# ZeningLin/ViBERTgrid-PyTorch

Measured on AMD Instinct MI355X. Metric: training docs/sec, 512x512 img + seq_len 512, bert-base+resnet34; 1/2/4/8 GPU, higher is better.
Workload: dtype f32

## Files before the change

vibertgrid-pytorch_amd/csrc/gemm_planes.hip:

```cpp
#include "vbg_common.h"
#include <type_traits>
#include <cstdlib>
#include <hip/hip_ext.h>
#include "../../include/vbg.h"

namespace vbg {

typedef unsigned pg_u32x4 __attribute__((ext_vector_type(4)));
typedef __bf16 pg_bf16x8 __attribute__((ext_vector_type(8)));
constexpr unsigned PG_INVALID = 0x80000000u;

__device__ __forceinline__ __amdgpu_buffer_rsrc_t pg_rsrc(const void* base) {
    return __builtin_amdgcn_make_buffer_rsrc(const_cast<void*>(base), 0, (int)0x80000000u, 0x00020000);
}

typedef _Float16 pg_f16x8 __attribute__((ext_vector_type(8)));
__device__ __forceinline__ void pg_split2(float a, float b, unsigned& hi, unsigned& lo) {
    typedef float f32x2_t __attribute__((ext_vector_type(2)));
    typedef _Float16 f16x2_t __attribute__((ext_vector_type(2)));
    const f32x2_t v = {a, b};
    const f16x2_t h = __builtin_convertvector(v, f16x2_t);
    const f16x2_t l = __builtin_convertvector((v - __builtin_convertvector(h, f32x2_t)) * 2048.f, f16x2_t);
    hi = __builtin_bit_cast(unsigned, h);
    lo = __builtin_bit_cast(unsigned, l);
// ... 336 lines not shown
            mma(fa1, fb1);
            __builtin_amdgcn_sched_barrier(0);
            asm volatile("s_waitcnt vmcnt(0) lgkmcnt(0)" ::: "memory");
            __builtin_amdgcn_s_barrier();
            __builtin_amdgcn_sched_barrier(0);
            read_frags(nxt, fo0, fa0, fb0);
        }
        __builtin_amdgcn_sched_barrier(0);
        settle0();
        cur = nxt;
    }
    }
    __syncthreads();

    const float* bias = p.bias;
    const bool add_bias = (bias != nullptr) && (split == 0);
    const int accumulate = p.accumulate, epi = p.epi;
    const bool atomic = accumulate && p.splitk > 1;
    float alpha = p.alpha;
    if constexpr (FORM) { if (a_amax) alpha *= vbg_pow2_scale(vbg_amax_read(a_amax)).y; }
    const long long ldc = ldc_;
    float* const C = pC;
    float* const C2 = p.C2;
    float* const Ct = reinterpret_cast<float*>(smem);
#pragma unroll
    for (int j = 0; j < TN; ++j)
#pragma unroll
        for (int i = 0; i < TM; ++i)
#pragma unroll
            for (int r = 0; r < 16; ++r)
                Ct[(wm * WM + i * 32 + (r & 3) + 8 * (r >> 2) + 4 * lk) * CTS + wn * WN + j * 32 + lr] =
                    (FORM == 1 ? acc[i][j][r] + acx[FORM == 1 ? i : 0][FORM == 1 ? j : 0][r] * (1.f / 2048.f) : acc[i][j][r]) * alpha;
    __syncthreads();
    constexpr int QN = BN / 4;
    unsigned short* const Cp = p.Cp;
    unsigned short* const Cq = p.Cq;
    float vmax = 0.f;
    float qsc = 1.f;
    if (Cq && p.cq_ref_in) {
        const float amx = __uint_as_float(vbg_amax_read(p.cq_ref_in));
        const float l1 = p.cq_l1_in ? __uint_as_float(*p.cq_l1_in) : 1.f;
        const float bound = amx * l1 * p.cq_mul;
        qsc = vbg_pow2_scale(__float_as_uint(bound)).x;
        if (p.cq_ref_out && pid == 0 && tid == 0) p.cq_ref_out[0] = __float_as_uint(bound);
    }
#pragma unroll
    for (int q = 0; q < BM * QN / NT; ++q) {
        const int idx = tid + q * NT;
        const int row = idx / QN, c = (idx % QN) * 4;
        const int gm = m0 + row, gn = n0 + c;
        if (gm >= M || gn >= N) continue;
        float4 v = *reinterpret_cast<const float4*>(&Ct[row * CTS + c]);
        if (add_bias) {
            const float4 b = *reinterpret_cast<const float4*>(bias + gn);
            v.x += b.x; v.y += b.y; v.z += b.z; v.w += b.w;
        }
        float* cp = C + (long long)gm * ldc + gn;
        if (atomic) {
            unsafeAtomicAdd(cp + 0, v.x); unsafeAtomicAdd(cp + 1, v.y); unsafeAtomicAdd(cp + 2, v.z); unsafeAtomicAdd(cp + 3, v.w);
            continue;
        }
        if (accumulate) {
            const float4 o = *reinterpret_cast<const float4*>(cp);
            v.x += o.x; v.y += o.y; v.z += o.z; v.w += o.w;
        }
        if (epi == VBG_EPI_RELU) v = make_float4(fmaxf(v.x, 0.f), fmaxf(v.y, 0.f), fmaxf(v.z, 0.f), fmaxf(v.w, 0.f));
        if (epi == VBG_EPI_MUL_GELU_GRAD) {
            const float4 hv = *reinterpret_cast<const float4*>(C2 + (long long)gm * ldc + gn);
            v.x *= gelu_erf_grad(hv.x); v.y *= gelu_erf_grad(hv.y); v.z *= gelu_erf_grad(hv.z); v.w *= gelu_erf_grad(hv.w);
        }
        if (C) *reinterpret_cast<float4*>(cp) = v;
        vmax = fmaxf(fmaxf(vmax, fmaxf(fabsf(v.x), fabsf(v.y))), fmaxf(fabsf(v.z), fabsf(v.w)));
        if (p.colsum) *reinterpret_cast<float4*>(&Ct[row * CTS + c]) = v;
        if (epi == VBG_EPI_GELU_DUAL) {
            v = make_float4(gelu_erf(v.x), gelu_erf(v.y), gelu_erf(v.z), gelu_erf(v.w));
            if (C2) *reinterpret_cast<float4*>(C2 + (long long)gm * ldc + gn) = v;
        }
        if (Cp) {
            const float e[4] = {v.x, v.y, v.z, v.w};
            unsigned short h[4], m[4], l[4];
#pragma unroll
            for (int t = 0; t < 4; ++t) {
                const unsigned u = __float_as_uint(e[t]);
                const float r1 = e[t] - __uint_as_float(u & 0xffff0000u);
                const unsigned u1 = __float_as_uint(r1);
                const float r2 = r1 - __uint_as_float(u1 & 0xffff0000u);
                h[t] = (unsigned short)(u >> 16); m[t] = (unsigned short)(u1 >> 16); l[t] = (unsigned short)(__float_as_uint(r2) >> 16);
            }
            unsigned short* o = Cp + (long long)gm * p.ldp + gn;
            *reinterpret_cast<uint2*>(o) = make_uint2(h[0] | ((unsigned)h[1] << 16), h[2] | ((unsigned)h[3] << 16));
            *reinterpret_cast<uint2*>(o + p.c_plane) = make_uint2(m[0] | ((unsigned)m[1] << 16), m[2] | ((unsigned)m[3] << 16));
            *reinterpret_cast<uint2*>(o + 2 * p.c_plane) = make_uint2(l[0] | ((unsigned)l[1] << 16), l[2] | ((unsigned)l[3] << 16));
        }
        if (Cq) {
            unsigned short* o = Cq + (long long)gm * p.ldq + gn;
            uint2 h, l;
            pg_split2(v.x * qsc, v.y * qsc, h.x, l.x);
            pg_split2(v.z * qsc, v.w * qsc, h.y, l.y);
            *reinterpret_cast<uint2*>(o) = h;
            *reinterpret_cast<uint2*>(o + p.q_plane) = l;
        }
    }
    if (p.colsum) {
        __syncthreads();
        if (tid < BN && n0 + tid < N) {
            float cs = 0.f;
            const int rows = min(BM, M - m0);
            for (int r = 0; r < rows; ++r) cs += Ct[r * CTS + tid];
            unsafeAtomicAdd(p.colsum + n0 + tid, cs);
        }
    }
    if (p.c_amax) {
        __syncthreads();
        vbg_amax_publish(vmax, p.c_amax, Ct);
    }
}

__device__ __forceinline__ void pg_split3(float x, unsigned short& h, unsigned short& m, unsigned short& l);

__global__ __launch_bounds__(512) void plane_gemm_256_kernel(const vbg_plane_gemm_desc p) {
    constexpr int BM = 256, BN = 256, WGN = 4, NW = 8, NT = 512, NST = 3, BK = 16;
    constexpr int WM = 128, WN = 64, TM = 4, TN = 2;
    constexpr int PA = BM * 32, PB = BN * 32;
    constexpr int STAGE = 3 * (PA + PB);
    constexpr int NIA = 3, NIB = 3;
    constexpr int CTS = BN + 4;
    constexpr int SMEM = NST * STAGE;
    static_assert(64 * CTS * 4 <= SMEM, "epilogue pass fits");
    __shared__ __attribute__((aligned(1024))) unsigned char smem[SMEM];

    const int tid = threadIdx.x, lane = tid & 63, wave = tid >> 6;
    const int M = p.M, N = p.N;
    const long long a_plane = p.a_plane, b_plane = p.b_plane, lda = p.lda, ldb = p.ldb;
    constexpr unsigned XCDS = 8, XCD_GROUP = 8;
    const unsigned gx = gridDim.x, gy = gridDim.y;
    const unsigned lin = blockIdx.x + gridDim.x * blockIdx.y;
    const unsigned total = gx * gy;
    const unsigned xcd = lin % XCDS, local = lin / XCDS;
    const unsigned per_xcd = (total + XCDS - 1) / XCDS, tall = (total % XCDS) ? (total % XCDS) : XCDS;
    const unsigned rem = xcd < tall ? xcd * per_xcd + local : tall * per_xcd + (xcd - tall) * (per_xcd - 1) + local;
    const unsigned band = XCD_GROUP * gy, bid = rem / band, first = bid * XCD_GROUP;
    const unsigned bm = min(gx - first, XCD_GROUP), inb = rem - bid * band;
    const unsigned tile_m = first + inb % bm, tile_n = inb / bm;
    const int m0 = (int)tile_m * BM, n0 = (int)tile_n * BN;
    if (m0 >= M || n0 >= N) return;
    const int ntiles = p.K / BK;

    unsigned avo[NIA], bvo[NIB];
    int alds[NIA], blds[NIB];
    {
        const int lrow = lane >> 1;
#pragma unroll
        for (int i = 0; i < NIA; ++i) {
            const int u = wave + NW * i, q = u / 8, rb = u % 8;
            const int r = rb * 32 + lrow;
            const int half = (lane & 1) ^ ((r >> 3) & 1);
            avo[i] = (m0 + r < M) ? (unsigned)(((long long)q * a_plane + (long long)r * lda) * 2 + half * 16) : PG_INVALID;
            alds[i] = __builtin_amdgcn_readfirstlane(q * PA + rb * 1024);
        }
#pragma unroll
        for (int i = 0; i < NIB; ++i) {
            const int u = wave + NW * i, q = u / 8, rb = u % 8;
            const int r = rb * 32 + lrow;
            const int half = (lane & 1) ^ ((r >> 3) & 1);
            bvo[i] = (n0 + r < N) ? (unsigned)(((long long)q * b_plane + (long long)r * ldb) * 2 + half * 16) : PG_INVALID;
            blds[i] = __builtin_amdgcn_readfirstlane(3 * PA + q * PB + rb * 1024);
        }
    }
    const unsigned short* abase = p.A + (long long)m0 * lda;
    const unsigned short* bbase = p.B + (long long)n0 * ldb;
    typedef __attribute__((address_space(3))) void* lds_ptr;
    auto issue = [&](int stage, unsigned inv) {
        unsigned char* sb = smem + stage * STAGE;
        const __amdgpu_buffer_rsrc_t ra = pg_rsrc(abase), rb = pg_rsrc(bbase);
#pragma unroll
        for (int i = 0; i < NIA; ++i)
            __builtin_amdgcn_raw_ptr_buffer_load_lds(ra, (lds_ptr)(sb + alds[i]), 16, (int)(avo[i] | inv), 0, 0, 0);
#pragma unroll
        for (int i = 0; i < NIB; ++i)
            __builtin_amdgcn_raw_ptr_buffer_load_lds(rb, (lds_ptr)(sb + blds[i]), 16, (int)(bvo[i] | inv), 0, 0, 0);
        abase += BK;
        bbase += BK;
    };

    const int wm = wave / WGN, wn = wave % WGN;
    const int lr = lane & 31, lk = lane >> 5;
    const int fo = lr * 32 + ((lk ^ ((lr >> 3) & 1)) << 4);
    f32x16 acc[TM][TN];
#pragma unroll
    for (int i = 0; i < TM; ++i)
#pragma unroll
        for (int j = 0; j < TN; ++j)
#pragma unroll
            for (int r = 0; r < 16; ++r) acc[i][j][r] = 0.f;
    pg_u32x4 fa[3][TM], fb[3][TN];
    auto read_frags = [&](int stage) {
        const unsigned char* as = smem + stage * STAGE + (wm * WM) * 32 + fo;
        const unsigned char* bs = smem + stage * STAGE + 3 * PA + (wn * WN) * 32 + fo;
        constexpr int order[3] = {2, 0, 1};
#pragma unroll
        for (int o = 0; o < 3; ++o) {
            const int q = order[o];
#pragma unroll
            for (int i = 0; i < TM; ++i) fa[q][i] = *reinterpret_cast<const pg_u32x4*>(as + q * PA + i * 32 * 32);
#pragma unroll
            for (int j = 0; j < TN; ++j) fb[q][j] = *reinterpret_cast<const pg_u32x4*>(bs + q * PB + j * 32 * 32);
        }
    };
    auto mma = [&]() {
        constexpr int qa[6] = {2, 0, 1, 1, 0, 0}, qb[6] = {0, 2, 1, 0, 1, 0};
#pragma unroll
        for (int t = 0; t < 6; ++t)
#pragma unroll
            for (int i = 0; i < TM; ++i)
#pragma unroll
                for (int j = 0; j < TN; ++j)
                    acc[i][j] = __builtin_amdgcn_mfma_f32_32x32x16_bf16(__builtin_bit_cast(pg_bf16x8, fa[qa[t]][i]),
                                                                        __builtin_bit_cast(pg_bf16x8, fb[qb[t]][j]), acc[i][j], 0, 0, 0);
    };
    constexpr int NIW = NIA + NIB;
    issue(0, 0u);
    issue(1, ntiles > 1 ? 0u : PG_INVALID);
    asm volatile("s_waitcnt vmcnt(%0)" ::"n"(NIW) : "memory");
    __builtin_amdgcn_s_barrier();
    int cur = 0;
    for (int t = 0; t < ntiles; ++t) {
        const int nxt = (cur + 1 == NST) ? 0 : cur + 1;
        const int nn = (nxt + 1 == NST) ? 0 : nxt + 1;
        issue(nn, t + 2 < ntiles ? 0u : PG_INVALID);
        read_frags(cur);
        mma();
        asm volatile("s_waitcnt vmcnt(%0) lgkmcnt(0)" ::"n"(NIW) : "memory");
        __builtin_amdgcn_s_barrier();
        cur = nxt;
    }
    __syncthreads();

    const float* bias = p.bias;
    const int epi = p.epi;
    const float alpha = p.alpha;
    const long long ldc = p.ldc;
    float* const C = p.C;
    float* const C2 = p.C2;
    unsigned short* const Cp = p.Cp;
    float* const Ct = reinterpret_cast<float*>(smem);
    constexpr int QN = BN / 4;
#pragma unroll
    for (int ps = 0; ps < 4; ++ps) {
        if (wm == (ps >> 1)) {
#pragma unroll
            for (int ii = 0; ii < 2; ++ii)
#pragma unroll
                for (int j = 0; j < TN; ++j)
#pragma unroll
                    for (int r = 0; r < 16; ++r)
                        Ct[(ii * 32 + (r & 3) + 8 * (r >> 2) + 4 * lk) * CTS + wn * WN + j * 32 + lr] = acc[2 * (ps & 1) + ii][j][r] * alpha;
        }
        __syncthreads();
#pragma unroll
        for (int q = 0; q < 64 * QN / NT; ++q) {
            const int idx = tid + q * NT;
            const int row = idx / QN, c = (idx % QN) * 4;
            const int gm = m0 + ps * 64 + row, gn = n0 + c;
            if (gm >= M || gn >= N) continue;
            float4 v = *reinterpret_cast<const float4*>(&Ct[row * CTS + c]);
            if (bias) {
                const float4 b = *reinterpret_cast<const float4*>(bias + gn);
                v.x += b.x; v.y += b.y; v.z += b.z; v.w += b.w;
            }
            float* cp = C + (long long)gm * ldc + gn;
            if (epi == VBG_EPI_RELU) v = make_float4(fmaxf(v.x, 0.f), fmaxf(v.y, 0.f), fmaxf(v.z, 0.f), fmaxf(v.w, 0.f));
            if (epi == VBG_EPI_MUL_GELU_GRAD) {
                const float4 hv = *reinterpret_cast<const float4*>(C2 + (long long)gm * ldc + gn);
                v.x *= gelu_erf_grad(hv.x); v.y *= gelu_erf_grad(hv.y); v.z *= gelu_erf_grad(hv.z); v.w *= gelu_erf_grad(hv.w);
            }
            if (C) *reinterpret_cast<float4*>(cp) = v;
            if (epi == VBG_EPI_GELU_DUAL) {
                v = make_float4(gelu_erf(v.x), gelu_erf(v.y), gelu_erf(v.z), gelu_erf(v.w));
                if (C2) *reinterpret_cast<float4*>(C2 + (long long)gm * ldc + gn) = v;
            }
            if (Cp) {
                const float e[4] = {v.x, v.y, v.z, v.w};
                unsigned short h[4], m[4], l[4];
#pragma unroll
                for (int t = 0; t < 4; ++t) pg_split3(e[t], h[t], m[t], l[t]);
                unsigned short* o = Cp + (long long)gm * p.ldp + gn;
                *reinterpret_cast<uint2*>(o) = make_uint2(h[0] | ((unsigned)h[1] << 16), h[2] | ((unsigned)h[3] << 16));
                *reinterpret_cast<uint2*>(o + p.c_plane) = make_uint2(m[0] | ((unsigned)m[1] << 16), m[2] | ((unsigned)m[3] << 16));
                *reinterpret_cast<uint2*>(o + 2 * p.c_plane) = make_uint2(l[0] | ((unsigned)l[1] << 16), l[2] | ((unsigned)l[3] << 16));
            }
        }
        __syncthreads();
    }
}

__device__ __forceinline__ void pg_split3(float x, unsigned short& h, unsigned short& m, unsigned short& l) {
    const unsigned u = __float_as_uint(x);
    const float r1 = x - __uint_as_float(u & 0xffff0000u);
    const unsigned u1 = __float_as_uint(r1);
    const float r2 = r1 - __uint_as_float(u1 & 0xffff0000u);
    h = (unsigned short)(u >> 16); m = (unsigned short)(u1 >> 16); l = (unsigned short)(__float_as_uint(r2) >> 16);
}

__global__ __launch_bounds__(256) void split_planes_kernel(const float* __restrict__ x, long long ldx, int rows, int cols,
                                                            unsigned short* __restrict__ out, int ldp, long long plane, int relu,
                                                            float* colsum) {
    extern __shared__ float sh_cols[];
    const int cpr = ldp / 8;
    const long long n = (long long)rows * cpr;
    const long long stride = (long long)gridDim.x * blockDim.x;
    float cs[8] = {0.f, 0.f, 0.f, 0.f, 0.f, 0.f, 0.f, 0.f};
    const long long i0 = (long long)blockIdx.x * blockDim.x + threadIdx.x;
    for (long long i = i0; i < n; i += stride) {
        const int r = (int)(i / cpr), c = (int)(i % cpr) * 8;
        float e[8];
        if (c + 8 <= cols && ((ldx & 3) == 0) && ((((uintptr_t)x) & 15) == 0)) {
            const float4 a = *reinterpret_cast<const float4*>(x + (long long)r * ldx + c);
            const float4 b = *reinterpret_cast<const float4*>(x + (long long)r * ldx + c + 4);
            e[0] = a.x; e[1] = a.y; e[2] = a.z; e[3] = a.w; e[4] = b.x; e[5] = b.y; e[6] = b.z; e[7] = b.w;
        } else {
#pragma unroll
            for (int t = 0; t < 8; ++t) e[t] = (c + t < cols) ? x[(long long)r * ldx + c + t] : 0.f;
        }
        unsigned short h[8], m[8], l[8];
#pragma unroll
        for (int t = 0; t < 8; ++t) {
            cs[t] += e[t];
            pg_split3(relu ? fmaxf(e[t], 0.f) : e[t], h[t], m[t], l[t]);
        }
        unsigned short* o = out + (long long)r * ldp + c;
        auto pack = [](const unsigned short* s) {
            return make_uint4(s[0] | ((unsigned)s[1] << 16), s[2] | ((unsigned)s[3] << 16), s[4] | ((unsigned)s[5] << 16), s[6] | ((unsigned)s[7] << 16));
        };
        *reinterpret_cast<uint4*>(o) = pack(h);
        *reinterpret_cast<uint4*>(o + plane) = pack(m);
        *reinterpret_cast<uint4*>(o + 2 * plane) = pack(l);
    }
    if (colsum) {
        for (int c = threadIdx.x; c < ldp; c += blockDim.x) sh_cols[c] = 0.f;
        __syncthreads();
        if (i0 < n) {
            const int c = (int)(i0 % cpr) * 8;
#pragma unroll
            for (int t = 0; t < 8; ++t) atomicAdd(&sh_cols[c + t], cs[t]);
        }
        __syncthreads();
        for (int c = threadIdx.x; c < cols; c += blockDim.x) {
            const float v = sh_cols[c];
            if (v != 0.f) unsafeAtomicAdd(colsum + c, v);
        }
    }
}

__global__ __launch_bounds__(256) void split_planes_pair_kernel(const float* __restrict__ x, long long ldx, int rows, int cols,
                                                                 unsigned short* __restrict__ out, int ldp, long long plane,
                                                                 const unsigned* amax, float* colsum) {
    extern __shared__ float sh_cols[];
    const float sc = amax ? vbg_pow2_scale(vbg_amax_read(amax)).x : 1.f;
    float cs[8] = {0.f, 0.f, 0.f, 0.f, 0.f, 0.f, 0.f, 0.f};
    const long long i0 = (long long)blockIdx.x * blockDim.x + threadIdx.x;
    const int cpr = ldp / 8;
    const long long n = (long long)rows * cpr;
    const long long stride = (long long)gridDim.x * blockDim.x;
    const bool vec = ((ldx & 3) == 0) && ((((uintptr_t)x) & 15) == 0);
    for (long long i = (long long)blockIdx.x * blockDim.x + threadIdx.x; i < n; i += stride) {
        const int r = (int)(i / cpr), c = (int)(i % cpr) * 8;
        float e[8];
        if (c + 8 <= cols && vec) {
            const float4 a = *reinterpret_cast<const float4*>(x + (long long)r * ldx + c);
            const float4 b = *reinterpret_cast<const float4*>(x + (long long)r * ldx + c + 4);
            e[0] = a.x; e[1] = a.y; e[2] = a.z; e[3] = a.w; e[4] = b.x; e[5] = b.y; e[6] = b.z; e[7] = b.w;
        } else {
#pragma unroll
            for (int t = 0; t < 8; ++t) e[t] = (c + t < cols) ? x[(long long)r * ldx + c + t] : 0.f;
        }
#pragma unroll
        for (int t = 0; t < 8; ++t) { cs[t] += e[t]; e[t] *= sc; }
        uint4 h, l;
        pg_split2(e[0], e[1], h.x, l.x); pg_split2(e[2], e[3], h.y, l.y); pg_split2(e[4], e[5], h.z, l.z); pg_split2(e[6], e[7], h.w, l.w);
        unsigned short* o = out + (long long)r * ldp + c;
        *reinterpret_cast<uint4*>(o) = h;
        *reinterpret_cast<uint4*>(o + plane) = l;
    }
    if (colsum) {
        for (int c = threadIdx.x; c < ldp; c += blockDim.x) sh_cols[c] = 0.f;
        __syncthreads();
        if (i0 < n) {
            const int c = (int)(i0 % cpr) * 8;
#pragma unroll
            for (int t = 0; t < 8; ++t) atomicAdd(&sh_cols[c + t], cs[t]);
        }
        __syncthreads();
        for (int c = threadIdx.x; c < cols; c += blockDim.x) {
            const float v = sh_cols[c];
            if (v != 0.f) unsafeAtomicAdd(colsum + c, v);
        }
    }
}

__global__ __launch_bounds__(256) void col_l1_max_kernel(const vbg_l1_entry* __restrict__ tab, unsigned* __restrict__ out) {
    const vbg_l1_entry e = tab[blockIdx.y];
    const int c0 = blockIdx.x * 64;
    if (c0 >= e.cols) return;
    const int tx = threadIdx.x & 15, ty = threadIdx.x >> 4;
    const int c = c0 + tx * 4;
    const bool vec = (e.ld & 3) == 0 && ((((uintptr_t)e.w) & 15) == 0) && c + 4 <= e.cols;
    float4 s = make_float4(0.f, 0.f, 0.f, 0.f);
#pragma unroll 4
    for (int r = ty; r < e.rows; r += 16) {
        const float* p = e.w + (long long)r * e.ld + c;
        if (vec) {
            const float4 v = *reinterpret_cast<const float4*>(p);
            s.x += fabsf(v.x); s.y += fabsf(v.y); s.z += fabsf(v.z); s.w += fabsf(v.w);
        } else {
            if (c < e.cols) s.x += fabsf(p[0]);
            if (c + 1 < e.cols) s.y += fabsf(p[1]);
            if (c + 2 < e.cols) s.z += fabsf(p[2]);
            if (c + 3 < e.cols) s.w += fabsf(p[3]);
        }
    }
    __shared__ float4 red[16][16];
    red[ty][tx] = s;
    __syncthreads();
    if (ty == 0) {
        float4 t = red[0][tx];
#pragma unroll
        for (int g = 1; g < 16; ++g) { const float4 v = red[g][tx]; t.x += v.x; t.y += v.y; t.z += v.z; t.w += v.w; }
        float m = fmaxf(fmaxf(t.x, t.y), fmaxf(t.z, t.w));
#pragma unroll
        for (int o = 8; o > 0; o >>= 1) m = fmaxf(m, __shfl_xor(m, o, 64));
        if (tx == 0) atomicMax(out + blockIdx.y, __float_as_uint(m));
    }
}

__global__ __launch_bounds__(256) void split_planes_t_kernel(const float* __restrict__ x, long long ldx, int rows, int cols,
                                                              unsigned short* __restrict__ out, int ldp, long long plane) {
    __shared__ float t[64][65];
    const int r0 = blockIdx.x * 64, c0 = blockIdx.y * 64;
    const int tid = threadIdx.x;
    const bool vec = ((ldx & 3) == 0) && ((((uintptr_t)x) & 15) == 0);
#pragma unroll
    for (int i = 0; i < 4; ++i) {
        const int f = tid + i * 256, r = f / 16, c = (f % 16) * 4;
        float4 v = make_float4(0.f, 0.f, 0.f, 0.f);
        if (r0 + r < rows) {
            const float* src = x + (long long)(r0 + r) * ldx + c0 + c;
            if (vec && c0 + c + 4 <= cols) v = *reinterpret_cast<const float4*>(src);
            else {
                if (c0 + c + 0 < cols) v.x = src[0];
                if (c0 + c + 1 < cols) v.y = src[1];
                if (c0 + c + 2 < cols) v.z = src[2];
                if (c0 + c + 3 < cols) v.w = src[3];
            }
        }
        t[r][c] = v.x; t[r][c + 1] = v.y; t[r][c + 2] = v.z; t[r][c + 3] = v.w;
    }
    __syncthreads();
#pragma unroll
    for (int i = 0; i < 2; ++i) {
        const int f = tid + i * 256, c = f / 8, rg = (f % 8) * 8;
        if (c0 + c >= cols || r0 + rg >= ldp) continue;
        unsigned short h[8], m[8], l[8];
#pragma unroll
        for (int e = 0; e < 8; ++e) pg_split3(t[rg + e][c], h[e], m[e], l[e]);
        unsigned short* o = out + (long long)(c0 + c) * ldp + r0 + rg;
        auto pack = [](const unsigned short* s) {
            return make_uint4(s[0] | ((unsigned)s[1] << 16), s[2] | ((unsigned)s[3] << 16), s[4] | ((unsigned)s[5] << 16), s[6] | ((unsigned)s[7] << 16));
        };
        *reinterpret_cast<uint4*>(o) = pack(h);
        *reinterpret_cast<uint4*>(o + plane) = pack(m);
        *reinterpret_cast<uint4*>(o + 2 * plane) = pack(l);
    }
}

template <bool PAIR>
__global__ __launch_bounds__(256) void split_planes_t_batched_kernel(const float* __restrict__ src, unsigned short* __restrict__ dst,
                                                                      const long long* __restrict__ tbl, int njobs, long long plane) {
    __shared__ float t[64][65];
    int j = 0;
    while (j + 1 < njobs && (long long)blockIdx.x >= tbl[(j + 1) * 6 + 5]) ++j;
    const long long* e = tbl + j * 6;
    const float* x = src + e[0];
    const int rows = (int)e[1], cols = (int)e[2], ldp = (int)e[4];
    unsigned short* out = dst + e[3];
    const int local = (int)(blockIdx.x - e[5]);
    const int tr = (ldp + 63) / 64;
    const int r0 = (local % tr) * 64, c0 = (local / tr) * 64;
    const int tid = threadIdx.x;
    const long long ldx = cols;
#pragma unroll
    for (int i = 0; i < 4; ++i) {
        const int f = tid + i * 256, r = f / 16, c = (f % 16) * 4;
        float v[4] = {0.f, 0.f, 0.f, 0.f};
        if (r0 + r < rows) {
#pragma unroll
            for (int q = 0; q < 4; ++q)
                if (c0 + c + q < cols) v[q] = x[(long long)(r0 + r) * ldx + c0 + c + q];
        }
        t[r][c] = v[0]; t[r][c + 1] = v[1]; t[r][c + 2] = v[2]; t[r][c + 3] = v[3];
    }
    __syncthreads();
#pragma unroll
    for (int i = 0; i < 2; ++i) {
        const int f = tid + i * 256, c = f / 8, rg = (f % 8) * 8;
        if (c0 + c >= cols || r0 + rg >= ldp) continue;
        unsigned short* o = out + (long long)(c0 + c) * ldp + r0 + rg;
        if constexpr (PAIR) {
            uint4 h, l;
            pg_split2(t[rg + 0][c], t[rg + 1][c], h.x, l.x); pg_split2(t[rg + 2][c], t[rg + 3][c], h.y, l.y);
            pg_split2(t[rg + 4][c], t[rg + 5][c], h.z, l.z); pg_split2(t[rg + 6][c], t[rg + 7][c], h.w, l.w);
            *reinterpret_cast<uint4*>(o) = h;
            *reinterpret_cast<uint4*>(o + plane) = l;
            continue;
        }
        unsigned short h[8], m[8], l[8];
#pragma unroll
        for (int q = 0; q < 8; ++q) pg_split3(t[rg + q][c], h[q], m[q], l[q]);
        auto pack = [](const unsigned short* s) {
            return make_uint4(s[0] | ((unsigned)s[1] << 16), s[2] | ((unsigned)s[3] << 16), s[4] | ((unsigned)s[5] << 16), s[6] | ((unsigned)s[7] << 16));
        };
        *reinterpret_cast<uint4*>(o) = pack(h);
        *reinterpret_cast<uint4*>(o + plane) = pack(m);
        *reinterpret_cast<uint4*>(o + 2 * plane) = pack(l);
    }
}

template <int BM, int BN, int WGM, int WGN, int NST, bool TRANS = false, int FORM = 1>
static void pg_launch_pair(const vbg_plane_gemm_desc& d, hipStream_t s, hipEvent_t e0, hipEvent_t e1) {
    dim3 g(cdiv(d.M, BM), cdiv(d.N, BN), 1);
    if (d.ngroups > 0) {
        int total = 0;
        for (int i = 0; i < d.ngroups; ++i) total += d.grp[i].tiles_m * d.grp[i].tiles_n;
        g = dim3(total, 1, 1);
    }
    (void)hipGetLastError();
    if (e0 && e1) hipExtLaunchKernelGGL((plane_gemm_kernel<BM, BN, WGM, WGN, NST, TRANS, FORM>), g, dim3(WGM * WGN * 64), 0, s, e0, e1, 0, d);
    else hipLaunchKernelGGL((plane_gemm_kernel<BM, BN, WGM, WGN, NST, TRANS, FORM>), g, dim3(WGM * WGN * 64), 0, s, d);
}

template <int BM, int BN, int WGM, int WGN, int NST, bool TRANS = false>
static void pg_launch(const vbg_plane_gemm_desc& d, hipStream_t s, hipEvent_t e0, hipEvent_t e1) {
    dim3 g(cdiv(d.M, BM), cdiv(d.N, BN), d.splitk);
    if (d.ngroups > 0) {
        int total = 0;
        for (int i = 0; i < d.ngroups; ++i) total += d.grp[i].tiles_m * d.grp[i].tiles_n;
        g = dim3(total, 1, d.splitk);
    }
    (void)hipGetLastError();
    if (e0 && e1) hipExtLaunchKernelGGL((plane_gemm_kernel<BM, BN, WGM, WGN, NST, TRANS>), g, dim3(WGM * WGN * 64), 0, s, e0, e1, 0, d);
    else hipLaunchKernelGGL((plane_gemm_kernel<BM, BN, WGM, WGN, NST, TRANS>), g, dim3(WGM * WGN * 64), 0, s, d);
}

}

using namespace vbg;

static int plane_gemm_dispatch(const vbg_plane_gemm_desc* desc, void* stream, void* e0, void* e1) {
    VBG_CHECK_ARG(desc != nullptr);
    vbg_plane_gemm_desc d = *desc;
    if (d.ngroups > 0) {
        VBG_CHECK_ARG(d.ngroups <= VBG_PLANE_MAX_GROUPS && d.Cp == nullptr && d.bias == nullptr && d.C2 == nullptr);
        for (int i = 0; i < d.ngroups; ++i) {
            vbg_plane_group& g = d.grp[i];
            VBG_CHECK_ARG(g.A && g.B && g.C && g.M > 0 && g.N > 0 && g.N % 4 == 0 && g.ldc % 4 == 0 && ((uintptr_t)g.C & 15) == 0);
            VBG_CHECK_ARG(((uintptr_t)g.A & 15) == 0 && ((uintptr_t)g.B & 15) == 0 && g.a_plane % 8 == 0 && g.b_plane % 8 == 0);
            if (d.trans) VBG_CHECK_ARG(g.lda % 32 == 0 && g.ldb % 32 == 0 && g.lda >= g.M && g.ldb >= g.N);
            else VBG_CHECK_ARG(g.lda % 8 == 0 && g.ldb % 8 == 0 && g.lda >= d.K && g.ldb >= d.K);
            VBG_CHECK_ARG(2 * g.a_plane * 2 + 256 * g.lda * 2 < 0x7fffffffll && 2 * g.b_plane * 2 + 256 * g.ldb * 2 < 0x7fffffffll);
            const int bn = (d.trans || d.tile != 64064) ? 128 : 64, bm = (d.trans && d.tile == 256128) ? 256 : bn;
            g.tiles_m = (g.M + bm - 1) / bm;
            g.tiles_n = (g.N + bn - 1) / bn;
        }
        d.A = d.grp[0].A; d.B = d.grp[0].B; d.C = d.grp[0].C; d.M = d.grp[0].M; d.N = d.grp[0].N;
        d.a_plane = d.grp[0].a_plane; d.b_plane = d.grp[0].b_plane; d.lda = d.grp[0].lda; d.ldb = d.grp[0].ldb; d.ldc = d.grp[0].ldc;
        if (!d.trans && d.tile != 64064) d.tile = 128129;
    }
    VBG_CHECK_ARG(d.A && d.B && (d.C || d.Cp || d.Cq));
    if (d.cq_ref_in) VBG_CHECK_ARG(d.Cq && d.cq_mul > 0.f && d.tile != 256256 && !d.trans && d.ngroups == 0 && d.splitk == 1);
    VBG_CHECK_ARG(d.M >= 0 && d.N >= 0 && d.K > 0);
    if (d.trans) VBG_CHECK_ARG(d.lda % 32 == 0 && d.ldb % 32 == 0 && d.lda >= d.M && d.ldb >= d.N);
    else VBG_CHECK_ARG(d.K % 32 == 0 && d.lda % 8 == 0 && d.ldb % 8 == 0 && d.lda >= d.K && d.ldb >= d.K);
    VBG_CHECK_ARG(((uintptr_t)d.A & 15) == 0 && ((uintptr_t)d.B & 15) == 0 && (d.a_plane % 8) == 0 && (d.b_plane % 8) == 0);
    VBG_CHECK_ARG(d.N % 4 == 0 && d.ldc % 4 == 0 && ((uintptr_t)d.C & 15) == 0 && ((uintptr_t)d.C2 & 15) == 0 && ((uintptr_t)d.bias & 15) == 0);
    VBG_CHECK_ARG(2 * d.a_plane * 2 + (long long)256 * d.lda * 2 < 0x7fffffffll && 2 * d.b_plane * 2 + (long long)256 * d.ldb * 2 < 0x7fffffffll);
    if (d.splitk < 1) d.splitk = 1;
    if (d.splitk > 1) VBG_CHECK_ARG(d.accumulate == 1 && d.C);
    if (d.accumulate) VBG_CHECK_ARG(d.epi == VBG_EPI_NONE && d.Cp == nullptr);
    if (d.colsum) VBG_CHECK_ARG(d.splitk == 1 && d.ngroups == 0 && !d.trans && !d.accumulate && d.epi != VBG_EPI_GELU_DUAL && d.tile != 256256);
    if (d.c_amax) VBG_CHECK_ARG(d.tile != 256256 && !d.trans && d.ngroups == 0 && d.splitk == 1);
    if (d.epi == VBG_EPI_GELU_DUAL) VBG_CHECK_ARG(d.C2 != nullptr || d.Cp != nullptr || d.Cq != nullptr);
    if (d.epi == VBG_EPI_MUL_GELU_GRAD) VBG_CHECK_ARG(d.C2 != nullptr && d.ngroups == 0 && !d.trans);
    if (d.Cp) VBG_CHECK_ARG(d.ldp % 8 == 0 && d.ldp >= d.N && ((uintptr_t)d.Cp & 7) == 0 && d.c_plane % 4 == 0);
    if (d.Cq) VBG_CHECK_ARG(d.ldq % 8 == 0 && d.ldq >= d.N && ((uintptr_t)d.Cq & 7) == 0 && d.q_plane % 4 == 0 && !d.accumulate && d.ngroups == 0 &&
                            !d.trans && d.tile != 256256);
    if (d.M == 0 || d.N == 0) return VBG_OK;
    hipStream_t s = (hipStream_t)stream;
    int tile = d.tile;
    if (d.form == 1 || d.form == 2) {
        VBG_CHECK_ARG(d.splitk == 1 && (d.ngroups == 0 || d.trans));
        hipEvent_t ev0 = (hipEvent_t)e0, ev1 = (hipEvent_t)e1;
        if (d.form == 2) {
            if (d.trans) {
                if (tile == 256128) pg_launch_pair<256, 128, 4, 2, 3, true, 2>(d, s, ev0, ev1);
                else pg_launch_pair<128, 128, 4, 2, 3, true, 2>(d, s, ev0, ev1);
            } else if (tile == 256128) pg_launch_pair<256, 128, 4, 2, 3, false, 2>(d, s, ev0, ev1);
            else if (tile == 128129 || tile == 0) pg_launch_pair<128, 128, 4, 2, 4, false, 2>(d, s, ev0, ev1);
            else if ((tile == 64064 || tile == 64004) && d.ngroups == 0 && !d.c_amax && !d.cq_ref_in && !d.colsum) {
                if (tile == 64004) pg_launch_pair<64, 64, 2, 2, 4, false, 2>(d, s, ev0, ev1);
                else pg_launch_pair<64, 64, 2, 2, 3, false, 2>(d, s, ev0, ev1);
            }
            else return VBG_EARG;
            VBG_LAUNCH_RET();
        }
        if (d.trans) {
            if (tile == 256128) pg_launch_pair<256, 128, 4, 2, 3, true>(d, s, ev0, ev1);
            else pg_launch_pair<128, 128, 4, 2, 3, true>(d, s, ev0, ev1);
            VBG_LAUNCH_RET();
        }
        if (tile == 256128) pg_launch_pair<256, 128, 4, 2, 3>(d, s, ev0, ev1);
        else if (tile == 128130) pg_launch_pair<128, 128, 2, 4, 3>(d, s, ev0, ev1);
        else if (tile == 128129 || tile == 0) pg_launch_pair<128, 128, 4, 2, 4>(d, s, ev0, ev1);
        else if ((tile == 64064 || tile == 64004) && d.ngroups == 0 && !d.c_amax && !d.cq_ref_in && !d.colsum) {
            if (tile == 64004) pg_launch_pair<64, 64, 2, 2, 4>(d, s, ev0, ev1);
            else pg_launch_pair<64, 64, 2, 2, 3>(d, s, ev0, ev1);
        } else return VBG_EARG;
        VBG_LAUNCH_RET();
    }
    VBG_CHECK_ARG(d.form == 0);
    if (d.trans) {
        if (tile == 256128) pg_launch<256, 128, 4, 2, 2, true>(d, s, (hipEvent_t)e0, (hipEvent_t)e1);
        else if (tile == 128130) pg_launch<128, 128, 2, 4, 3, true>(d, s, (hipEvent_t)e0, (hipEvent_t)e1);
        else pg_launch<128, 128, 4, 2, 3, true>(d, s, (hipEvent_t)e0, (hipEvent_t)e1);
        VBG_LAUNCH_RET();
    }
    if (tile == 0) {
        const long t128 = (long)cdiv(d.M, 128) * cdiv(d.N, 128) * d.splitk;
        tile = (t128 >= 200 && d.N >= 128) ? 128128 : 64064;
    }
    if (tile == 256256) {
        VBG_CHECK_ARG(d.splitk == 1 && !d.accumulate && d.K % 16 == 0);
        const dim3 g(cdiv(d.M, 256), cdiv(d.N, 256));
        (void)hipGetLastError();
        hipEvent_t ev0 = (hipEvent_t)e0, ev1 = (hipEvent_t)e1;
        if (ev0 && ev1) hipExtLaunchKernelGGL(plane_gemm_256_kernel, g, dim3(512), 0, s, ev0, ev1, 0, d);
        else hipLaunchKernelGGL(plane_gemm_256_kernel, g, dim3(512), 0, s, d);
        VBG_LAUNCH_RET();
    }
    if (tile == 256128) pg_launch<256, 128, 4, 2, 2>(d, s, (hipEvent_t)e0, (hipEvent_t)e1);
    else if (tile == 128128) pg_launch<128, 128, 2, 2, 3>(d, s, (hipEvent_t)e0, (hipEvent_t)e1);
    else if (tile == 128129) pg_launch<128, 128, 4, 2, 3>(d, s, (hipEvent_t)e0, (hipEvent_t)e1);
    else if (tile == 128130) pg_launch<128, 128, 2, 4, 3>(d, s, (hipEvent_t)e0, (hipEvent_t)e1);
    else if (tile == 128064) pg_launch<128, 64, 2, 2, 3>(d, s, (hipEvent_t)e0, (hipEvent_t)e1);
    else if (tile == 64064) pg_launch<64, 64, 2, 2, 3>(d, s, (hipEvent_t)e0, (hipEvent_t)e1);
    else return VBG_EARG;
    VBG_LAUNCH_RET();
}

extern "C" int vbg_plane_gemm(const vbg_plane_gemm_desc* desc, void* stream) { return plane_gemm_dispatch(desc, stream, nullptr, nullptr); }

extern "C" int vbg_plane_gemm_timed(const vbg_plane_gemm_desc* desc, void* stream, void* start_event, void* stop_event) {
    VBG_CHECK_ARG(start_event && stop_event);
    return plane_gemm_dispatch(desc, stream, start_event, stop_event);
}

extern "C" int vbg_split_planes(const float* x, long long ldx, int rows, int cols, unsigned short* out, int ldp, long long plane,
                                int relu, float* colsum_accum, void* stream) {
    VBG_CHECK_ARG(rows >= 0 && cols >= 0 && ldp % 32 == 0 && ldp >= cols && plane >= (long long)rows * ldp && plane % 8 == 0);
    if (rows == 0 || cols == 0) return VBG_OK;
    VBG_CHECK_ARG(x && out && ((uintptr_t)out & 15) == 0);
    const long long n = (long long)rows * (ldp / 8);
    long long g = (n + 255) / 256;
    size_t lds = 0;
    if (colsum_accum) {
        VBG_CHECK_ARG(relu == 0 && ldp * 4 <= 64 * 1024);
        const long long cpr = ldp / 8;
        long long a = cpr, b = 256;
        while (b) { const long long t = a % b; a = b; b = t; }
        const long long unit = cpr / a;
        long long k = 288 / unit;
        if (k < 1) k = 1;
        const long long need = (g + unit - 1) / unit;
        if (k > need) k = need;
        g = k * unit;
        lds = (size_t)ldp * 4;
    } else if (g > 256 * 16) {
        g = 256 * 16;
    }
    VBG_LAUNCH(split_planes_kernel, dim3((unsigned)g), dim3(256), lds, (hipStream_t)stream, x, ldx, rows, cols, out, ldp, plane, relu,
               colsum_accum);
    VBG_LAUNCH_RET();
}

extern "C" int vbg_split_planes_pair(const float* x, long long ldx, int rows, int cols, unsigned short* out, int ldp, long long plane,
                                     const unsigned* amax, float* colsum_accum, void* stream) {
    VBG_CHECK_ARG(rows >= 0 && cols >= 0 && ldp % 32 == 0 && ldp >= cols && plane >= (long long)rows * ldp && plane % 8 == 0);
    if (rows == 0 || cols == 0) return VBG_OK;
    VBG_CHECK_ARG(x && out && ((uintptr_t)out & 15) == 0);
    const long long n = (long long)rows * (ldp / 8);
    long long g = (n + 255) / 256;
    size_t lds = 0;
    if (colsum_accum) {
        VBG_CHECK_ARG(ldp * 4 <= 64 * 1024);
        const long long cpr = ldp / 8;
        long long a = cpr, b = 256;
        while (b) { const long long t = a % b; a = b; b = t; }
        const long long unit = cpr / a;
        long long k = 288 / unit;
        if (k < 1) k = 1;
        const long long need = (g + unit - 1) / unit;
        if (k > need) k = need;
        g = k * unit;
        lds = (size_t)ldp * 4;
    } else if (g > 256 * 16) {
        g = 256 * 16;
    }
    VBG_LAUNCH(split_planes_pair_kernel, dim3((unsigned)g), dim3(256), lds, (hipStream_t)stream, x, ldx, rows, cols, out, ldp, plane, amax, colsum_accum);
    VBG_LAUNCH_RET();
}

extern "C" int vbg_col_l1_max(const vbg_l1_entry* table_dev, int n, int max_cols, unsigned* out, void* stream) {
    VBG_CHECK_ARG(n >= 0 && max_cols >= 0);
    if (n == 0 || max_cols == 0) return VBG_OK;
    VBG_CHECK_ARG(table_dev && out);
    VBG_LAUNCH(col_l1_max_kernel, dim3((unsigned)((max_cols + 63) / 64), (unsigned)n), dim3(256), 0, (hipStream_t)stream, table_dev, out);
    VBG_LAUNCH_RET();
}

extern "C" int vbg_split_planes_t(const float* x, long long ldx, int rows, int cols, unsigned short* out, int ldp, long long plane,
                                  void* stream) {
    VBG_CHECK_ARG(rows >= 0 && cols >= 0 && ldp % 32 == 0 && ldp >= rows && plane >= (long long)cols * ldp && plane % 8 == 0);
    if (rows == 0 || cols == 0) return VBG_OK;
    VBG_CHECK_ARG(x && out && ((uintptr_t)out & 15) == 0);
    VBG_LAUNCH(split_planes_t_kernel, dim3(cdiv(ldp, 64), cdiv(cols, 64)), dim3(256), 0, (hipStream_t)stream, x, ldx, rows, cols, out, ldp, plane);
    VBG_LAUNCH_RET();
}

extern "C" int vbg_split_planes_t_batched(const float* src, unsigned short* dst, const long long* tbl_dev, int njobs, int total_tiles,
                                          long long plane, void* stream) {
    VBG_CHECK_ARG(njobs >= 0 && total_tiles >= 0);
    if (njobs == 0 || total_tiles == 0) return VBG_OK;
    VBG_CHECK_ARG(src && dst && tbl_dev && ((uintptr_t)dst & 15) == 0 && plane % 8 == 0);
    VBG_LAUNCH(split_planes_t_batched_kernel<false>, dim3(total_tiles), dim3(256), 0, (hipStream_t)stream, src, dst, tbl_dev, njobs, plane);
    VBG_LAUNCH_RET();
}

extern "C" int vbg_split_planes_pair_t_batched(const float* src, unsigned short* dst, const long long* tbl_dev, int njobs, int total_tiles,
                                               long long plane, void* stream) {
    VBG_CHECK_ARG(njobs >= 0 && total_tiles >= 0);
    if (njobs == 0 || total_tiles == 0) return VBG_OK;
    VBG_CHECK_ARG(src && dst && tbl_dev && ((uintptr_t)dst & 15) == 0 && plane % 8 == 0);
    VBG_LAUNCH(split_planes_t_batched_kernel<true>, dim3(total_tiles), dim3(256), 0, (hipStream_t)stream, src, dst, tbl_dev, njobs, plane);
    VBG_LAUNCH_RET();
}
```

Baseline: 248.4.

## Use 2D column-tiled kernel for split-planes with fused column sums

Adds a dedicated kernel for the split-planes paths that also accumulate column sums. It uses a 2D grid where each block owns 256 columns and a slab of rows, unrolls four rows of loads per thread, and reduces partial sums through a fixed shared-memory tile before issuing one global atomic per column. The old path used a grid-stride loop with a gcd-derived grid size and per-element shared atomics. The new layout removes shared atomic contention and the odd grid sizing, at the cost of more blocks doing global atomics on colsum.

```diff
diff --git a/vibertgrid-pytorch_amd/csrc/gemm_planes.hip b/vibertgrid-pytorch_amd/csrc/gemm_planes.hip
--- a/vibertgrid-pytorch_amd/csrc/gemm_planes.hip
+++ b/vibertgrid-pytorch_amd/csrc/gemm_planes.hip
@@ -662,63 +662,37 @@
     h = (unsigned short)(u >> 16); m = (unsigned short)(u1 >> 16); l = (unsigned short)(__float_as_uint(r2) >> 16);
 }
 
+__device__ __forceinline__ void pg_load8(const float* __restrict__ x, long long ldx, int r, int c, int cols, bool vec, float (&e)[8]) {
+    if (c + 8 <= cols && vec) {
+        const float4 a = *reinterpret_cast<const float4*>(x + (long long)r * ldx + c);
+        const float4 b = *reinterpret_cast<const float4*>(x + (long long)r * ldx + c + 4);
+        e[0] = a.x; e[1] = a.y; e[2] = a.z; e[3] = a.w; e[4] = b.x; e[5] = b.y; e[6] = b.z; e[7] = b.w;
+    } else {
+#pragma unroll
+        for (int t = 0; t < 8; ++t) e[t] = (c + t < cols) ? x[(long long)r * ldx + c + t] : 0.f;
+    }
+}
+__device__ __forceinline__ void pg_store8_bf16x3(const float (&e)[8], int relu, unsigned short* __restrict__ o, long long plane) {
+    unsigned short h[8], m[8], l[8];
+#pragma unroll
+    for (int t = 0; t < 8; ++t) pg_split3(relu ? fmaxf(e[t], 0.f) : e[t], h[t], m[t], l[t]);
+    auto pack = [](const unsigned short* s) {
+        return make_uint4(s[0] | ((unsigned)s[1] << 16), s[2] | ((unsigned)s[3] << 16), s[4] | ((unsigned)s[5] << 16), s[6] | ((unsigned)s[7] << 16));
+    };
+    *reinterpret_cast<uint4*>(o) = pack(h);
+    *reinterpret_cast<uint4*>(o + plane) = pack(m);
+    *reinterpret_cast<uint4*>(o + 2 * plane) = pack(l);
+}
+__device__ __forceinline__ void pg_store8_pair(const float (&e)[8], float sc, unsigned short* __restrict__ o, long long plane) {
+    uint4 h, l;
+    pg_split2(e[0] * sc, e[1] * sc, h.x, l.x); pg_split2(e[2] * sc, e[3] * sc, h.y, l.y);
+    pg_split2(e[4] * sc, e[5] * sc, h.z, l.z); pg_split2(e[6] * sc, e[7] * sc, h.w, l.w);
+    *reinterpret_cast<uint4*>(o) = h;
+    *reinterpret_cast<uint4*>(o + plane) = l;
+}
+
 __global__ __launch_bounds__(256) void split_planes_kernel(const float* __restrict__ x, long long ldx, int rows, int cols,
-                                                            unsigned short* __restrict__ out, int ldp, long long plane, int relu,
-                                                            float* colsum) {
-    extern __shared__ float sh_cols[];
-    const int cpr = ldp / 8;
-    const long long n = (long long)rows * cpr;
-    const long long stride = (long long)gridDim.x * blockDim.x;
-    float cs[8] = {0.f, 0.f, 0.f, 0.f, 0.f, 0.f, 0.f, 0.f};
-    const long long i0 = (long long)blockIdx.x * blockDim.x + threadIdx.x;
-    for (long long i = i0; i < n; i += stride) {
-        const int r = (int)(i / cpr), c = (int)(i % cpr) * 8;
-        float e[8];
-        if (c + 8 <= cols && ((ldx & 3) == 0) && ((((uintptr_t)x) & 15) == 0)) {
-            const float4 a = *reinterpret_cast<const float4*>(x + (long long)r * ldx + c);
-            const float4 b = *reinterpret_cast<const float4*>(x + (long long)r * ldx + c + 4);
-            e[0] = a.x; e[1] = a.y; e[2] = a.z; e[3] = a.w; e[4] = b.x; e[5] = b.y; e[6] = b.z; e[7] = b.w;
-        } else {
-#pragma unroll
-            for (int t = 0; t < 8; ++t) e[t] = (c + t < cols) ? x[(long long)r * ldx + c + t] : 0.f;
-        }
-        unsigned short h[8], m[8], l[8];
-#pragma unroll
-        for (int t = 0; t < 8; ++t) {
-            cs[t] += e[t];
-            pg_split3(relu ? fmaxf(e[t], 0.f) : e[t], h[t], m[t], l[t]);
-        }
-        unsigned short* o = out + (long long)r * ldp + c;
-        auto pack = [](const unsigned short* s) {
-            return make_uint4(s[0] | ((unsigned)s[1] << 16), s[2] | ((unsigned)s[3] << 16), s[4] | ((unsigned)s[5] << 16), s[6] | ((unsigned)s[7] << 16));
-        };
-        *reinterpret_cast<uint4*>(o) = pack(h);
-        *reinterpret_cast<uint4*>(o + plane) = pack(m);
-        *reinterpret_cast<uint4*>(o + 2 * plane) = pack(l);
-    }
-    if (colsum) {
-        for (int c = threadIdx.x; c < ldp; c += blockDim.x) sh_cols[c] = 0.f;
-        __syncthreads();
-        if (i0 < n) {
-            const int c = (int)(i0 % cpr) * 8;
-#pragma unroll
-            for (int t = 0; t < 8; ++t) atomicAdd(&sh_cols[c + t], cs[t]);
-        }
-        __syncthreads();
-        for (int c = threadIdx.x; c < cols; c += blockDim.x) {
-            const float v = sh_cols[c];
-            if (v != 0.f) unsafeAtomicAdd(colsum + c, v);
-        }
-    }
-}
-
-__global__ __launch_bounds__(256) void split_planes_pair_kernel(const float* __restrict__ x, long long ldx, int rows, int cols,
-                                                                 unsigned short* __restrict__ out, int ldp, long long plane,
-                                                                 const unsigned* amax, float* colsum) {
-    extern __shared__ float sh_cols[];
-    const float sc = amax ? vbg_pow2_scale(vbg_amax_read(amax)).x : 1.f;
-    float cs[8] = {0.f, 0.f, 0.f, 0.f, 0.f, 0.f, 0.f, 0.f};
-    const long long i0 = (long long)blockIdx.x * blockDim.x + threadIdx.x;
+                                                            unsigned short* __restrict__ out, int ldp, long long plane, int relu) {
     const int cpr = ldp / 8;
     const long long n = (long long)rows * cpr;
     const long long stride = (long long)gridDim.x * blockDim.x;
@@ -726,35 +700,83 @@
     for (long long i = (long long)blockIdx.x * blockDim.x + threadIdx.x; i < n; i += stride) {
         const int r = (int)(i / cpr), c = (int)(i % cpr) * 8;
         float e[8];
-        if (c + 8 <= cols && vec) {
-            const float4 a = *reinterpret_cast<const float4*>(x + (long long)r * ldx + c);
-            const float4 b = *reinterpret_cast<const float4*>(x + (long long)r * ldx + c + 4);
-            e[0] = a.x; e[1] = a.y; e[2] = a.z; e[3] = a.w; e[4] = b.x; e[5] = b.y; e[6] = b.z; e[7] = b.w;
-        } else {
-#pragma unroll
-            for (int t = 0; t < 8; ++t) e[t] = (c + t < cols) ? x[(long long)r * ldx + c + t] : 0.f;
-        }
-#pragma unroll
-        for (int t = 0; t < 8; ++t) { cs[t] += e[t]; e[t] *= sc; }
-        uint4 h, l;
-        pg_split2(e[0], e[1], h.x, l.x); pg_split2(e[2], e[3], h.y, l.y); pg_split2(e[4], e[5], h.z, l.z); pg_split2(e[6], e[7], h.w, l.w);
+        pg_load8(x, ldx, r, c, cols, vec, e);
+        pg_store8_bf16x3(e, relu, out + (long long)r * ldp + c, plane);
+    }
+}
+
+__global__ __launch_bounds__(256) void split_planes_pair_kernel(const float* __restrict__ x, long long ldx, int rows, int cols,
+                                                                 unsigned short* __restrict__ out, int ldp, long long plane,
+                                                                 const unsigned* amax) {
+    const float sc = amax ? vbg_pow2_scale(vbg_amax_read(amax)).x : 1.f;
+    const int cpr = ldp / 8;
+    const long long n = (long long)rows * cpr;
+    const long long stride = (long long)gridDim.x * blockDim.x;
+    const bool vec = ((ldx & 3) == 0) && ((((uintptr_t)x) & 15) == 0);
+    for (long long i = (long long)blockIdx.x * blockDim.x + threadIdx.x; i < n; i += stride) {
+        const int r = (int)(i / cpr), c = (int)(i % cpr) * 8;
+        float e[8];
+        pg_load8(x, ldx, r, c, cols, vec, e);
+        pg_store8_pair(e, sc, out + (long long)r * ldp + c, plane);
+    }
+}
+
+constexpr int SPLIT_CS_ROWS = 32, SPLIT_CS_UNROLL = 4;
+template <bool PAIR>
+__global__ __launch_bounds__(256) void split_planes_colsum_kernel(const float* __restrict__ x, long long ldx, int rows, int cols,
+                                                                   unsigned short* __restrict__ out, int ldp, long long plane,
+                                                                   const unsigned* amax, float* colsum, int rows_per_block) {
+    __shared__ float red[8][256 + 8];
+    const int tx = threadIdx.x & 31, ty = threadIdx.x >> 5;
+    const int c = ((int)blockIdx.x * 32 + tx) * 8;
+    const bool live = c < ldp;
+    const long long rb = (long long)blockIdx.y * rows_per_block;
+    const int r0 = (int)rb, r1 = (int)(rb + rows_per_block < rows ? rb + rows_per_block : rows);
+    const float sc = (PAIR && amax) ? vbg_pow2_scale(vbg_amax_read(amax)).x : 1.f;
+    const bool vec = ((ldx & 3) == 0) && ((((uintptr_t)x) & 15) == 0);
+    float cs[8] = {0.f, 0.f, 0.f, 0.f, 0.f, 0.f, 0.f, 0.f};
+    auto take = [&](const float (&e)[8], int r) {
+#pragma unroll
+        for (int t = 0; t < 8; ++t) cs[t] += e[t];
         unsigned short* o = out + (long long)r * ldp + c;
-        *reinterpret_cast<uint4*>(o) = h;
-        *reinterpret_cast<uint4*>(o + plane) = l;
-    }
-    if (colsum) {
-        for (int c = threadIdx.x; c < ldp; c += blockDim.x) sh_cols[c] = 0.f;
-        __syncthreads();
-        if (i0 < n) {
-            const int c = (int)(i0 % cpr) * 8;
-#pragma unroll
-            for (int t = 0; t < 8; ++t) atomicAdd(&sh_cols[c + t], cs[t]);
-        }
-        __syncthreads();
-        for (int c = threadIdx.x; c < cols; c += blockDim.x) {
-            const float v = sh_cols[c];
-            if (v != 0.f) unsafeAtomicAdd(colsum + c, v);
-        }
+        if constexpr (PAIR) pg_store8_pair(e, sc, o, plane);
+        else pg_store8_bf16x3(e, 0, o, plane);
+    };
+    if (live) {
+        const bool fast = vec && c + 8 <= cols;
+        for (int r = r0 + ty; r < r1; r += 8 * SPLIT_CS_UNROLL) {
+            if (fast && r + 8 * (SPLIT_CS_UNROLL - 1) < r1) {
+                float4 a[SPLIT_CS_UNROLL], b[SPLIT_CS_UNROLL];
+#pragma unroll
+                for (int u = 0; u < SPLIT_CS_UNROLL; ++u) {
+                    const float* px = x + (long long)(r + 8 * u) * ldx + c;
+                    a[u] = *reinterpret_cast<const float4*>(px);
+                    b[u] = *reinterpret_cast<const float4*>(px + 4);
+                }
+                __builtin_amdgcn_sched_barrier(0);
+#pragma unroll
+                for (int u = 0; u < SPLIT_CS_UNROLL; ++u) {
+                    const float e[8] = {a[u].x, a[u].y, a[u].z, a[u].w, b[u].x, b[u].y, b[u].z, b[u].w};
+                    take(e, r + 8 * u);
+                }
+            } else {
+                for (int u = 0; u < SPLIT_CS_UNROLL && r + 8 * u < r1; ++u) {
+                    float e[8];
+                    pg_load8(x, ldx, r + 8 * u, c, cols, vec, e);
+                    take(e, r + 8 * u);
+                }
+            }
+        }
+    }
+    *reinterpret_cast<float4*>(&red[ty][tx * 8]) = make_float4(cs[0], cs[1], cs[2], cs[3]);
+    *reinterpret_cast<float4*>(&red[ty][tx * 8 + 4]) = make_float4(cs[4], cs[5], cs[6], cs[7]);
+    __syncthreads();
+    const int col = (int)blockIdx.x * 256 + threadIdx.x;
+    if (col < cols) {
+        float v = red[0][threadIdx.x];
+#pragma unroll
+        for (int g = 1; g < 8; ++g) v += red[g][threadIdx.x];
+        if (v != 0.f) unsafeAtomicAdd(colsum + col, v);
     }
 }
 
@@ -1023,31 +1045,33 @@
     return plane_gemm_dispatch(desc, stream, start_event, stop_event);
 }
 
+namespace {
+inline void split_colsum_grid(int rows, int ldp, dim3& grid, int& rows_per_block) {
+    long long rpb = vbg::SPLIT_CS_ROWS;
+    while ((rows + rpb - 1) / rpb > 65535) rpb *= 2;
+    rows_per_block = (int)rpb;
+    grid = dim3((unsigned)((ldp / 8 + 31) / 32), (unsigned)((rows + rpb - 1) / rpb));
+}
+}
+
 extern "C" int vbg_split_planes(const float* x, long long ldx, int rows, int cols, unsigned short* out, int ldp, long long plane,
                                 int relu, float* colsum_accum, void* stream) {
     VBG_CHECK_ARG(rows >= 0 && cols >= 0 && ldp % 32 == 0 && ldp >= cols && plane >= (long long)rows * ldp && plane % 8 == 0);
     if (rows == 0 || cols == 0) return VBG_OK;
     VBG_CHECK_ARG(x && out && ((uintptr_t)out & 15) == 0);
+    if (colsum_accum) {
+        VBG_CHECK_ARG(relu == 0);
+        dim3 grid;
+        int rpb;
+        split_colsum_grid(rows, ldp, grid, rpb);
+        VBG_LAUNCH(split_planes_colsum_kernel<false>, grid, dim3(256), 0, (hipStream_t)stream, x, ldx, rows, cols, out, ldp, plane,
+                   (const unsigned*)nullptr, colsum_accum, rpb);
+        VBG_LAUNCH_RET();
+    }
     const long long n = (long long)rows * (ldp / 8);
     long long g = (n + 255) / 256;
-    size_t lds = 0;
-    if (colsum_accum) {
-        VBG_CHECK_ARG(relu == 0 && ldp * 4 <= 64 * 1024);
-        const long long cpr = ldp / 8;
-        long long a = cpr, b = 256;
-        while (b) { const long long t = a % b; a = b; b = t; }
-        const long long unit = cpr / a;
-        long long k = 288 / unit;
-        if (k < 1) k = 1;
-        const long long need = (g + unit - 1) / unit;
-        if (k > need) k = need;
-        g = k * unit;
-        lds = (size_t)ldp * 4;
-    } else if (g > 256 * 16) {
-        g = 256 * 16;
-    }
-    VBG_LAUNCH(split_planes_kernel, dim3((unsigned)g), dim3(256), lds, (hipStream_t)stream, x, ldx, rows, cols, out, ldp, plane, relu,
-               colsum_accum);
+    if (g > 256 * 16) g = 256 * 16;
+    VBG_LAUNCH(split_planes_kernel, dim3((unsigned)g), dim3(256), 0, (hipStream_t)stream, x, ldx, rows, cols, out, ldp, plane, relu);
     VBG_LAUNCH_RET();
 }
 
@@ -1056,25 +1080,18 @@
     VBG_CHECK_ARG(rows >= 0 && cols >= 0 && ldp % 32 == 0 && ldp >= cols && plane >= (long long)rows * ldp && plane % 8 == 0);
     if (rows == 0 || cols == 0) return VBG_OK;
     VBG_CHECK_ARG(x && out && ((uintptr_t)out & 15) == 0);
+    if (colsum_accum) {
+        dim3 grid;
+        int rpb;
+        split_colsum_grid(rows, ldp, grid, rpb);
+        VBG_LAUNCH(split_planes_colsum_kernel<true>, grid, dim3(256), 0, (hipStream_t)stream, x, ldx, rows, cols, out, ldp, plane, amax,
+                   colsum_accum, rpb);
+        VBG_LAUNCH_RET();
+    }
     const long long n = (long long)rows * (ldp / 8);
     long long g = (n + 255) / 256;
-    size_t lds = 0;
-    if (colsum_accum) {
-        VBG_CHECK_ARG(ldp * 4 <= 64 * 1024);
-        const long long cpr = ldp / 8;
-        long long a = cpr, b = 256;
-        while (b) { const long long t = a % b; a = b; b = t; }
-        const long long unit = cpr / a;
-        long long k = 288 / unit;
-        if (k < 1) k = 1;
-        const long long need = (g + unit - 1) / unit;
-        if (k > need) k = need;
-        g = k * unit;
-        lds = (size_t)ldp * 4;
-    } else if (g > 256 * 16) {
-        g = 256 * 16;
-    }
-    VBG_LAUNCH(split_planes_pair_kernel, dim3((unsigned)g), dim3(256), lds, (hipStream_t)stream, x, ldx, rows, cols, out, ldp, plane, amax, colsum_accum);
+    if (g > 256 * 16) g = 256 * 16;
+    VBG_LAUNCH(split_planes_pair_kernel, dim3((unsigned)g), dim3(256), 0, (hipStream_t)stream, x, ldx, rows, cols, out, ldp, plane, amax);
     VBG_LAUNCH_RET();
 }
 
```

New measurement: 245.4. 0.988x the previous value.
